# aanna0701/face-recognition-pytorch

Measured on AMD Instinct MI355X. Metric: train imgs/sec IR-50-layout ResNet50 + ArcFace/PartialFC head, 112x112, higher is better.
Workload: dtype bf16

## Files before the change

face-recognition-pytorch_amd/frhip/csrc/head.hip:

```cpp
#include "igemm_nt.h"
#include "margin_shared.h"
#include "frhip.h"

namespace frhip {

struct MarginConstEx : MarginConst { float m3, thr; };

constexpr int MG_ARC = 0, MG_ARC_EASY = 1, MG_COS = 2, MG_ROWS = 3;
struct MarginRows { float s, eps; const float* m_ang; const float* m_add; };
template <int MK, bool FILT> struct MarginArgOf { typedef MarginConstEx type; };
template <> struct MarginArgOf<MG_ARC, false> { typedef MarginConst type; };
template <> struct MarginArgOf<MG_ROWS, false> { typedef MarginRows type; };
template <int MK, bool FILT>
using MarginArg = typename MarginArgOf<MK, FILT>::type;

template <typename T>
__global__ __launch_bounds__(256) void l2norm_rows_kernel(const float* __restrict__ x, T* __restrict__ xhat,
                                                          float* __restrict__ norms, int rows, int D, float eps) {
    const int row = blockIdx.x * 4 + (threadIdx.x >> 6), lane = threadIdx.x & 63;
    if (row >= rows) return;
    const float* xr = x + (size_t)row * D;
    float ss = 0.f;
    for (int j = lane * 4; j < D; j += 256) {
        const f32x4_t v = *reinterpret_cast<const f32x4_t*>(xr + j);
// ... 124 lines not shown
                    if (cls == lab && mrow) {
                        ztarget[m] = zz;
                        if constexpr (SUB) tsub[m] = (int)((win[nt] >> (2 * (4 * mt + e))) & 3u);
                    }
                } else {
                    float d = 0.f;
                    if (cls < g.Nout && mrow) {
                        const float p = __expf(zz - gm) * gs;
                        bool inside;
                        if constexpr (MK == MG_ROWS) inside = raw >= tlo && raw <= thi;
                        else inside = raw >= -1.f && raw <= 1.f && !filtered;
                        d = inside ? (p - (cls == lab ? 1.f : 0.f)) * gscale * mc.s * slope : 0.f;
                    }
                    acc[nt][mt][e] = d;
                }
            }
        if (FWD) {
            vmax = lane_max_bit5(lane_max_bit4(vmax));
            float vs = 0.f;
            const float vref = vmax == -INFINITY ? 0.f : vmax;
#pragma unroll
            for (int nt = 0; nt < 4; ++nt)
#pragma unroll
                for (int e = 0; e < 4; ++e) vs += __expf(z[nt][e] - vref);
            vs = lane_sum_bit5(lane_sum_bit4(vs));
            if (fg == 0 && mrow) {
                part_max[(size_t)group * g.M + m] = vmax;
                part_sum[(size_t)group * g.M + m] = vs;
            }
        }
    }
}

template <typename T>
__device__ __forceinline__ void head_store_tile(const NtGeom& g, NtMainloop<T, 2, 2>& ml, char* smem, int m0, int n0, T* o, int ldt,
                                                int ncols, T* ot, int ldtt) {
    constexpr int P = NtTile<T, 2, 2>::template stage_pitch<T>();
    constexpr int EPV = 16 / (int)sizeof(T), LPR = 64 / EPV, RPI = 64 / LPR;
    const char* mine = ml.template stage_out<T>(smem);
    const int lane = lane_id(), chunk = lane % LPR, rsub = lane / LPR;
    const int n = n0 + chunk * EPV;
    for (int it = 0; it < 64 / RPI; ++it) {
        const int row = it * RPI + rsub, m = m0 + row;
        if (m < g.M && n < ncols)
            *reinterpret_cast<Vec16<T>*>(o + (size_t)m * ldt + n) = *reinterpret_cast<const Vec16<T>*>(mine + row * P + chunk * 16);
    }
    if (ot) {
        const int cls = n0 + lane;
        if (cls < g.Nout) {
#pragma unroll
            for (int v = 0; v < 64 / EPV; ++v) {
                Vec16<T> tv;
#pragma unroll
                for (int e = 0; e < EPV; ++e) tv.v[e] = *reinterpret_cast<const T*>(mine + (v * EPV + e) * P + lane * (int)sizeof(T));
                const int mcol = m0 + v * EPV;
                if (mcol < ldtt) *reinterpret_cast<Vec16<T>*>(ot + (size_t)cls * ldtt + mcol) = tv;
            }
        }
    }
}

template <typename T, bool FWD, int MK, bool FILT>
__global__ __launch_bounds__(256, 2) void head_kernel(NtGeom g, const void* __restrict__ ehat,
                                                             const void* __restrict__ what, const int* __restrict__ labels,
                                                             MarginArg<MK, FILT> mc, float* __restrict__ part_max,
                                                             float* __restrict__ part_sum, float* __restrict__ ztarget,
                                                             const float* __restrict__ rowmax, const float* __restrict__ rowsum,
                                                             float gscale, const float* __restrict__ upstream,
                                                             void* __restrict__ dt, int ldt, void* __restrict__ dtt, int ldtt,
                                                             int mtiles, int ntiles) {
    typedef NtTile<T, 2, 2> Tile;
    extern __shared__ __attribute__((aligned(16))) char smem[];
    const uint32_t lin = xcd_remap(blockIdx.x, gridDim.x);
    const int mtile = (int)(lin % (uint32_t)mtiles), ntile = (int)(lin / (uint32_t)mtiles);
    NtMainloop<T, 2, 2> ml;
    ml.run(g, ehat, what, smem, mtile, ntile, 0, g.ksteps);

    const int lane = lane_id(), wave = wave_id();
    const int wm = wave >> 1, wn = wave & 1;
    const int m0 = mtile * Tile::BM + wm * 64, n0 = ntile * Tile::BN + wn * 64;
    head_epilogue<FWD, MK, FILT, false>(lane, g, ml.acc, nullptr, m0, n0, ntile * 2 + wn, labels, mc, part_max, part_sum, ztarget, nullptr,
                                        rowmax, rowsum, gscale, upstream);
    if (!FWD) head_store_tile<T>(g, ml, smem, m0, n0, reinterpret_cast<T*>(dt), ldt, ldt, reinterpret_cast<T*>(dtt), ldtt);
}

constexpr int HEAD_SUB_MAX = 4;

template <typename T, bool FWD, int MK, bool FILT>
__global__ __launch_bounds__(256, 2) void head_sub_kernel(NtGeom g, const void* __restrict__ ehat,
                                                                 const void* __restrict__ what, const int* __restrict__ labels,
                                                                 MarginArg<MK, FILT> mc, int K, float* __restrict__ part_max,
                                                                 float* __restrict__ part_sum, float* __restrict__ ztarget,
                                                                 int* __restrict__ tsub, const float* __restrict__ rowmax,
                                                                 const float* __restrict__ rowsum, float gscale,
                                                                 const float* __restrict__ upstream, void* __restrict__ dt, int ldt,
                                                                 int ldp, void* __restrict__ dtt, int ldtt, int mtiles, int ntiles) {
    typedef NtTile<T, 2, 2> Tile;
    extern __shared__ __attribute__((aligned(16))) char smem[];
    const uint32_t lin = xcd_remap(blockIdx.x, gridDim.x);
    const int mtile = (int)(lin % (uint32_t)mtiles), ntile = (int)(lin / (uint32_t)mtiles);
    NtMainloop<T, 2, 2> ml;
    f32x4_t best[4][4];
    uint32_t win[4] = {0u, 0u, 0u, 0u};
    for (int k = 0; k < K; ++k) {
        if (k) __syncthreads();
        ml.run(g, ehat, reinterpret_cast<const char*>(what) + (size_t)k * g.b_bytes, smem, mtile, ntile, 0, g.ksteps);
#pragma unroll
        for (int nt = 0; nt < 4; ++nt)
#pragma unroll
            for (int mt = 0; mt < 4; ++mt)
#pragma unroll
                for (int e = 0; e < 4; ++e) {
                    const float v = ml.acc[nt][mt][e];
                    if (k == 0) best[nt][mt][e] = v;
                    else if (v > best[nt][mt][e]) {
                        best[nt][mt][e] = v;
                        win[nt] = (win[nt] & ~(3u << (2 * (4 * mt + e)))) | ((uint32_t)k << (2 * (4 * mt + e)));
                    }
                }
    }

    const int lane = lane_id(), wave = wave_id();
    const int wm = wave >> 1, wn = wave & 1;
    const int m0 = mtile * Tile::BM + wm * 64, n0 = ntile * Tile::BN + wn * 64;
    head_epilogue<FWD, MK, FILT, true>(lane, g, best, win, m0, n0, ntile * 2 + wn, labels, mc, part_max, part_sum, ztarget, tsub, rowmax,
                                       rowsum, gscale, upstream);
    if (!FWD)
        for (int k = 0; k < K; ++k) {
#pragma unroll
            for (int nt = 0; nt < 4; ++nt)
#pragma unroll
                for (int mt = 0; mt < 4; ++mt)
#pragma unroll
                    for (int e = 0; e < 4; ++e)
                        ml.acc[nt][mt][e] = ((win[nt] >> (2 * (4 * mt + e))) & 3u) == (uint32_t)k ? best[nt][mt][e] : 0.f;
            head_store_tile<T>(g, ml, smem, m0, n0, reinterpret_cast<T*>(dt) + (size_t)k * ldp, ldt, ldp,
                               dtt ? reinterpret_cast<T*>(dtt) + (size_t)k * g.Nout * ldtt : nullptr, ldtt);
        }
}

__global__ __launch_bounds__(256) void head_rowreduce_kernel(const float* __restrict__ part_max, const float* __restrict__ part_sum,
                                                             int ngroups, int N, float* __restrict__ rowmax, float* __restrict__ rowsum) {
    __shared__ float smax[16][17], ssum[16][17];
    const int ml = threadIdx.x & 15, gl = threadIdx.x >> 4;
    const int m = blockIdx.x * 16 + ml;
    float mx = -INFINITY, s = 0.f;
    if (m < N) {
        for (int gq = gl; gq < ngroups; gq += 16) {
            const float pm = part_max[(size_t)gq * N + m], ps = part_sum[(size_t)gq * N + m];
            if (pm > mx) { s = s * __expf(mx - pm) + ps; mx = pm; }
            else if (pm > -INFINITY) s += ps * __expf(pm - mx);
        }
    }
    smax[gl][ml] = mx; ssum[gl][ml] = s;
    __syncthreads();
    if (gl == 0 && m < N) {
        float M = -INFINITY;
#pragma unroll
        for (int k = 0; k < 16; ++k) M = fmaxf(M, smax[k][ml]);
        float S = 0.f;
#pragma unroll
        for (int k = 0; k < 16; ++k) if (smax[k][ml] > -INFINITY) S += ssum[k][ml] * __expf(smax[k][ml] - M);
        rowmax[m] = M; rowsum[m] = S;
    }
}

__global__ void head_rescale_kernel(float* __restrict__ rowsum, const float* __restrict__ local_max,
                                    const float* __restrict__ global_max, int N) {
    const int m = blockIdx.x * blockDim.x + threadIdx.x;
    if (m < N) rowsum[m] *= __expf(local_max[m] - global_max[m]);
}

__global__ void head_target_prob_kernel(const float* __restrict__ ztarget, const int* __restrict__ labels,
                                        const float* __restrict__ rowmax, const float* __restrict__ rowsum,
                                        float* __restrict__ q, int N) {
    const int m = blockIdx.x * blockDim.x + threadIdx.x;
    if (m < N) q[m] = labels[m] >= 0 ? __expf(ztarget[m] - rowmax[m]) / rowsum[m] : 0.f;
}

__global__ void head_pack_stats_kernel(const float* __restrict__ ztarget, const int* __restrict__ labels,
                                       const float* __restrict__ rowmax, const float* __restrict__ rowsum,
                                       float* __restrict__ packed, int N) {
    const int m = blockIdx.x * blockDim.x + threadIdx.x;
    if (m < N) {
// ... 20 lines not shown

__global__ void head_loss_kernel(const float* __restrict__ q, int N, float* __restrict__ loss) {
    __shared__ float red[256];
    float acc = 0.f;
    for (int m = threadIdx.x; m < N; m += 256) acc += logf(fmaxf(q[m], 1e-30f));
    red[threadIdx.x] = acc;
    __syncthreads();
    for (int d = 128; d > 0; d >>= 1) { if (threadIdx.x < d) red[threadIdx.x] += red[threadIdx.x + d]; __syncthreads(); }
    if (threadIdx.x == 0) loss[0] = -red[0] / (float)N;
}

struct HeadMargin { int mk; bool filt; MarginConstEx ex; MarginRows rows; };

template <int MK, bool FILT>
static MarginArg<MK, FILT> margin_arg(const HeadMargin& hm) {
    if constexpr (MK == MG_ROWS) return hm.rows;
    else return hm.ex;
}

struct HeadArgs {
    const void *ehat, *what;
    const int* labels;
    float *pmax, *psum, *zt;
    int* tsub;
    const float *rmax, *rsum;
    float gscale;
    const float* upstream;
    void* dt;
    int ldt, ldp;
    void* dtt;
    int ldtt;
};

template <typename T, bool FWD, int MK, bool FILT>
static int head_launch_mk(const NtGeom& g, const HeadArgs& a, const HeadMargin& hm, int K, hipStream_t stream) {
    typedef NtTile<T, 2, 2> Tile;
    const int mtiles = (g.M + Tile::BM - 1) / Tile::BM, ntiles = (g.Nout + Tile::BN - 1) / Tile::BN;
    const int lds = Tile::template lds_bytes<T>();
    const MarginArg<MK, FILT> mc = margin_arg<MK, FILT>(hm);
    auto plain = head_kernel<T, FWD, MK, FILT>;
    auto sub = head_sub_kernel<T, FWD, MK, FILT>;
    const char* who = K ? "head_sub" : "head";
    if (set_dynamic_lds(K ? reinterpret_cast<const void*>(sub) : reinterpret_cast<const void*>(plain), lds, who)) return FRHIP_ELAUNCH;
    if (K)
        hipLaunchKernelGGL(sub, dim3(mtiles * ntiles), dim3(256), lds, stream, g, a.ehat, a.what, a.labels, mc, K, a.pmax, a.psum, a.zt,
                           a.tsub, a.rmax, a.rsum, a.gscale, a.upstream, a.dt, a.ldt, a.ldp, a.dtt, a.ldtt, mtiles, ntiles);
    else
        hipLaunchKernelGGL(plain, dim3(mtiles * ntiles), dim3(256), lds, stream, g, a.ehat, a.what, a.labels, mc, a.pmax, a.psum, a.zt,
                           a.rmax, a.rsum, a.gscale, a.upstream, a.dt, a.ldt, a.dtt, a.ldtt, mtiles, ntiles);
    return check_launch(who);
}

template <bool FWD>
static int head_launch(int dtype, const NtGeom& g, const HeadArgs& a, const HeadMargin& hm, int K, hipStream_t stream) {
#define HEAD_VARIANT(MKV, FV) \
    if (hm.mk == MKV && hm.filt == FV) \
        return dtype == FRHIP_DT_BF16 ? head_launch_mk<bf16_t, FWD, MKV, FV>(g, a, hm, K, stream) \
                                      : head_launch_mk<float, FWD, MKV, FV>(g, a, hm, K, stream);
    HEAD_VARIANT(MG_ARC, false)
    HEAD_VARIANT(MG_ARC, true)
    HEAD_VARIANT(MG_ARC_EASY, false)
    HEAD_VARIANT(MG_ARC_EASY, true)
    HEAD_VARIANT(MG_COS, false)
    HEAD_VARIANT(MG_COS, true)
    HEAD_VARIANT(MG_ROWS, false)
#undef HEAD_VARIANT
    set_error("head: unknown margin variant %d", hm.mk);
    return FRHIP_EINVAL;
}

static int head_geom(NtGeom& g, int dtype, int n, int cl, int d, bool sub, int K, const char* who) {
    if (sub && (K < 1 || K > HEAD_SUB_MAX)) {
        set_error("%s: %d sub-centres per class (1 .. %d are supported)", who, K, HEAD_SUB_MAX);
        return FRHIP_EINVAL;
    }
    const int es = dtype == FRHIP_DT_BF16 ? 2 : 4, bke = NT_ROWB / es;
    if ((dtype != FRHIP_DT_BF16 && dtype != FRHIP_DT_F32) || n <= 0 || cl <= 0 || d <= 0 || (d % bke)) {
        set_error("%s: unsupported shape/dtype (n=%d classes=%d d=%d dtype=%d; d must be a multiple of %d)", who, n, cl, d, dtype, bke);
        return FRHIP_EINVAL;
    }
    if (1LL * cl * d * es > 0x7fffffffLL || 1LL * n * d * es > 0x7fffffffLL) { set_error("%s: operand exceeds 2 GiB", who); return FRHIP_EINVAL; }
    if (sub && 1LL * K * cl * d * es > 0x7fffffffLL) { set_error("%s: %d planes of %d classes exceed 2 GiB", who, K, cl); return FRHIP_EINVAL; }
    g.H = 1; g.W = 1; g.C = d; g.Ho = 1; g.Wo = 1; g.R = 1; g.S = 1; g.stride = 1; g.pad = 0; g.mode = 0;
    g.M = n; g.Nout = cl; g.Ktot = d; g.ksteps = d / bke; g.ksteps_per_split = g.ksteps;
    g.a_bytes = (uint32_t)(1LL * n * d * es); g.b_bytes = (uint32_t)(1LL * cl * d * es);
    g.par_a = -1; g.par_b = -1; g.hc = 0; g.wc = 0; g.par_r0 = 0; g.par_s0 = 0;
    return FRHIP_OK;
}

static int head_pitches(int dtype, int n, int cl, bool sub, int K, int ldt, int ldp, const void* dtt, int ldtt, const char* who) {
    const int epv = dtype == FRHIP_DT_BF16 ? 8 : 4;
    if (sub && (ldp < cl || (ldp % epv) || 1LL * ldt < 1LL * K * ldp || (ldt % epv))) {
        set_error("%s: bad dT pitches (row pitch %d, plane pitch %d, %d planes of %d classes)", who, ldt, ldp, K, cl);
        return FRHIP_EINVAL;
    }
    if (!sub && (ldt < cl || (ldt % epv))) { set_error("%s: bad dT pitch %d", who, ldt); return FRHIP_EINVAL; }
    if (dtt && (ldtt < n || (ldtt % epv))) { set_error("%s: bad transposed pitch %d", who, ldtt); return FRHIP_EINVAL; }
    return FRHIP_OK;
}

static int margin_desc(const frhip_margin_t* mg, HeadMargin& hm, const char* who) {
    if (!margin_desc_ok(mg)) {
        set_error("%s: bad margin descriptor (kind=%d thr=%g)", who, mg ? mg->kind : -1, mg ? (double)mg->filter_thr : 0.0);
        return FRHIP_EINVAL;
    }
    const bool arc = mg->kind == FRHIP_MARGIN_ARCFACE;
    static_cast<MarginConst&>(hm.ex) = margin_const(mg->s, arc ? mg->m : 0.f);
    hm.ex.m3 = arc ? 0.f : mg->m;
    hm.ex.thr = mg->filter_thr;
    hm.mk = arc ? (mg->easy ? MG_ARC_EASY : MG_ARC) : MG_COS;
    hm.filt = mg->filter_thr > 0.f;
    return FRHIP_OK;
}

static int margin_desc(const frhip_margin_rows_t* mg, HeadMargin& hm, const char* who) {
    if (!margin_rows_desc_ok(mg)) {
        set_error("%s: bad per-row margin descriptor (null pointer, or eps outside (0, 0.5))", who);
        return FRHIP_EINVAL;
    }
    hm.rows.s = mg->s; hm.rows.eps = mg->eps; hm.rows.m_ang = mg->m_ang; hm.rows.m_add = mg->m_add;
    hm.mk = MG_ROWS;
    hm.filt = false;
    return FRHIP_OK;
}

template <typename D>
static int head_fwd_impl(const char* who, int dtype, const void* ehat, const void* what, const int* labels, int n, int classes, int d,
                         bool sub, int K, const D* margin, float* part_max, float* part_sum, float* ztarget, int* tsub, float* rowmax,
                         float* rowsum, hipStream_t stream) {
    NtGeom g;
    HeadMargin hm = {};
    int rc = head_geom(g, dtype, n, classes, d, sub, K, who);
    if (rc || (rc = margin_desc(margin, hm, who))) return rc;
    HeadArgs a = {};
    a.ehat = ehat; a.what = what; a.labels = labels; a.pmax = part_max; a.psum = part_sum; a.zt = ztarget; a.tsub = tsub;
    if ((rc = head_launch<true>(dtype, g, a, hm, sub ? K : 0, stream))) return rc;
    hipLaunchKernelGGL(head_rowreduce_kernel, dim3((n + 15) / 16), dim3(256), 0, stream, part_max, part_sum,
                       frhip_head_groups(classes), n, rowmax, rowsum);
    char tag[64];
    snprintf(tag, sizeof(tag), "%s/rowreduce", who);
    return check_launch(tag);
}

template <typename D>
static int head_bwd_dt_impl(const char* who, int dtype, const void* ehat, const void* what, const int* labels, int n, int classes, int d,
                            bool sub, int K, const D* margin, const float* rowmax, const float* rowsum, float gscale,
                            const float* upstream, void* dt, int ldt, int ldp, void* dtt, int ldtt, hipStream_t stream) {
    NtGeom g;
    HeadMargin hm = {};
    int rc = head_geom(g, dtype, n, classes, d, sub, K, who);
    if (rc || (rc = head_pitches(dtype, n, classes, sub, K, ldt, ldp, dtt, ldtt, who)) || (rc = margin_desc(margin, hm, who))) return rc;
    HeadArgs a = {};
    a.ehat = ehat; a.what = what; a.labels = labels; a.rmax = rowmax; a.rsum = rowsum; a.gscale = gscale; a.upstream = upstream;
    a.dt = dt; a.ldt = ldt; a.ldp = ldp; a.dtt = dtt; a.ldtt = ldtt;
    return head_launch<false>(dtype, g, a, hm, sub ? K : 0, stream);
}

__device__ __forceinline__ double block_sum_f64(double v, double* red) {
#pragma unroll
    for (int d = 1; d < 64; d <<= 1) v += __shfl_xor(v, d);
    __syncthreads();
    if ((threadIdx.x & 63) == 0) red[threadIdx.x >> 6] = v;
    __syncthreads();
    double r = 0.0;
    for (int w = 0; w < (int)(blockDim.x >> 6); ++w) r += red[w];
    return r;
}

__device__ __forceinline__ double safe_norm(float x) { return (double)fminf(fmaxf(x, 0.001f), 100.f); }

__global__ __launch_bounds__(1024) void adaface_margins_kernel(const float* __restrict__ norms, int n, double m, double h, double t_alpha,
                                                               double eps, int update, float* __restrict__ batch_mean,
                                                               float* __restrict__ batch_std, float* __restrict__ m_ang,
                                                               float* __restrict__ m_add) {
// ... 3 lines not shown
    const double mean = block_sum_f64(acc, red) / (double)n;
    acc = 0.0;
    for (int i = threadIdx.x; i < n; i += blockDim.x) {
        const double dv = safe_norm(norms[i]) - mean;
        acc += dv * dv;
    }
    const double sd = sqrt(block_sum_f64(acc, red) / (double)(n - 1));
    double bm = (double)batch_mean[0], bs = (double)batch_std[0];
    if (update) { bm = t_alpha * mean + (1.0 - t_alpha) * bm; bs = t_alpha * sd + (1.0 - t_alpha) * bs; }
    __syncthreads();
    if (update && threadIdx.x == 0) { batch_mean[0] = (float)bm; batch_std[0] = (float)bs; }
    for (int i = threadIdx.x; i < n; i += blockDim.x) {
        const double k = fmin(fmax(h * (safe_norm(norms[i]) - bm) / (bs + eps), -1.0), 1.0);
        m_ang[i] = (float)(-m * k);
        m_add[i] = (float)(m + m * k);
    }
}

}

using namespace frhip;

extern "C" int frhip_adaface_margins(const float* norms, int n, double m, double h, double t_alpha, double eps, int update,
                                     float* batch_mean, float* batch_std, float* m_ang, float* m_add, hipStream_t stream) {
    if (n < 2 || !norms || !batch_mean || !batch_std || !m_ang || !m_add) {
        set_error("frhip_adaface_margins: needs n >= 2 norms (n=%d) and non-null norms, batch_mean, batch_std, m_ang, m_add", n);
        return FRHIP_EINVAL;
    }
    hipLaunchKernelGGL(adaface_margins_kernel, dim3(1), dim3(n > 256 ? 1024 : 256), 0, stream, norms, n, m, h, t_alpha, eps, update,
                       batch_mean, batch_std, m_ang, m_add);
    return check_launch("frhip_adaface_margins");
}

extern "C" int frhip_head_sub_max(void) { return HEAD_SUB_MAX; }

extern "C" int frhip_head_groups(int num_classes) { return ((num_classes + 127) / 128) * 2; }

extern "C" int frhip_head_fwd_ex(int dtype, const void* ehat, const void* what, const int* labels, int n, int classes,
                                 int d, const frhip_margin_t* margin, float* part_max, float* part_sum, float* ztarget,
                                 float* rowmax, float* rowsum, hipStream_t stream) {
    return head_fwd_impl("frhip_head_fwd", dtype, ehat, what, labels, n, classes, d, false, 1, margin, part_max, part_sum, ztarget, nullptr,
                         rowmax, rowsum, stream);
}

extern "C" int frhip_head_fwd(int dtype, const void* ehat, const void* what, const int* labels, int n, int classes,
                              int d, float s, float m, float* part_max, float* part_sum, float* ztarget,
                              float* rowmax, float* rowsum, hipStream_t stream) {
    const frhip_margin_t mg = {FRHIP_MARGIN_ARCFACE, 0, s, m, 0.f};
    return frhip_head_fwd_ex(dtype, ehat, what, labels, n, classes, d, &mg, part_max, part_sum, ztarget, rowmax, rowsum, stream);
}

extern "C" int frhip_head_fwd_rows(int dtype, const void* ehat, const void* what, const int* labels, int n, int classes,
                                   int d, const frhip_margin_rows_t* margin, float* part_max, float* part_sum, float* ztarget,
                                   float* rowmax, float* rowsum, hipStream_t stream) {
    return head_fwd_impl("frhip_head_fwd_rows", dtype, ehat, what, labels, n, classes, d, false, 1, margin, part_max, part_sum, ztarget,
                         nullptr, rowmax, rowsum, stream);
}

extern "C" int frhip_head_fwd_sub(int dtype, const void* ehat, const void* what, const int* labels, int n, int classes, int d,
                                  int subcenters, const frhip_margin_t* margin, float* part_max, float* part_sum, float* ztarget,
                                  int* tsub, float* rowmax, float* rowsum, hipStream_t stream) {
    return head_fwd_impl("frhip_head_fwd_sub", dtype, ehat, what, labels, n, classes, d, true, subcenters, margin, part_max, part_sum,
                         ztarget, tsub, rowmax, rowsum, stream);
}

extern "C" int frhip_head_fwd_sub_rows(int dtype, const void* ehat, const void* what, const int* labels, int n, int classes, int d,
// ... 90 lines not shown
```

include/frhip.h:

```cpp
#ifndef FRHIP_H
#define FRHIP_H
#include <stddef.h>
#include <stdint.h>

#ifdef __cplusplus
extern "C" {
#endif

#ifndef FRHIP_STREAM_T
#define FRHIP_STREAM_T
#ifdef __HIP_PLATFORM_AMD__
#include <hip/hip_runtime_api.h>
typedef hipStream_t frhip_stream_t;
#else
typedef void* frhip_stream_t;
#endif
#endif

#define FRHIP_OK 0
#define FRHIP_EINVAL (-1)
#define FRHIP_ELAUNCH (-2)
#define FRHIP_DT_BF16 0
#define FRHIP_DT_F32 1

const char* frhip_last_error(void);
int frhip_abi_version(void);
int frhip_spin(long long ticks, frhip_stream_t stream);

int frhip_nt_block_m(int k);
int frhip_conv_stat_rows(int dtype, int m, int k, int h, int w, int c, int r, int s, int stride, int pad);
int frhip_set_wgrad_taps9(int enabled);
int frhip_set_conv_halo(int enabled);
int frhip_set_halo_wide_dirs(int dirs);
int frhip_set_epi_lean(int enabled);
int frhip_set_ew_batch(int enabled);
int frhip_set_nt_tile(int tile);
int frhip_conv_fwd_affine(int dtype, const void* x, const void* w, void* y, const float* scale, const float* shift, int relu,
                          const void* residual, int n, int h, int wd, int c, int k, int r, int s, int stride, int pad,
                          frhip_stream_t stream);
int frhip_conv_fwd(int dtype, const void* x, const void* w, void* y, float* stats_partial,
                   int n, int h, int wd, int c, int k, int r, int s, int stride, int pad, frhip_stream_t stream);
int frhip_conv_dgrad(int dtype, const void* dy, const void* wt, void* dx, const void* residual,
                     int n, int h, int wd, int c, int k, int r, int s, int stride, int pad, frhip_stream_t stream);
int frhip_dgrad_stat_rows(int dtype, int n, int h, int wd, int c, int k, int r, int s, int stride, int pad);
int frhip_conv_dgrad_bnred(int dtype, const void* dy, const void* wt, void* dx, const void* residual,
                           const void* y_bn, const float* mean, const float* invstd, const float* mask_scale,
                           const float* mask_shift, float* stats_partial, int n, int h, int wd, int c, int k,
                           int r, int s, int stride, int pad, frhip_stream_t stream);
int frhip_conv_dgrad_fused(int dtype, const void* dy, const void* wt, void* dx, const void* residual, int residual_stride,
                           const void* y_bn, const float* mean, const float* invstd, const float* mask_scale,
                           const float* mask_shift, float* stats_partial, int n, int h, int wd, int c, int k,
                           int r, int s, int stride, int pad, frhip_stream_t stream);
int frhip_conv_dgrad_fused_rs(int dtype, const void* dy, const void* wt, void* dx, const void* residual, int residual_stride,
                              const void* y_bn, const float* mean, const float* invstd, const float* mask_scale,
                              const float* mask_shift, const float* rowscale, int rows_per, float keep_scale,
                              float* stats_partial, int n, int h, int wd, int c, int k, int r, int s, int stride, int pad,
                              frhip_stream_t stream);
int frhip_conv_wgrad(int dtype, const void* dy, const void* x, float* dw, int n, int h, int w, int c,
                     int k, int r, int s, int stride, int pad, int splits, float* workspace, size_t workspace_bytes,
                     frhip_stream_t stream);
int frhip_conv_wgrad_chain_ok(int dtype, int n, int h, int w, int c, int k, int r, int s, int stride, int pad);
int frhip_conv_wgrad_chain(int dtype, const void* dy, const void* x, int n, int h, int w, int c, int k, float* slabs,
                           size_t slab_bytes, float* prev_dw, const float* prev_slabs, int prev_k, int prev_c, int prev_splits,
                           int* splits_out, frhip_stream_t stream);
int frhip_conv_wgrad_chain_finish(float* dw, float* slabs, int k, int c, int splits, frhip_stream_t stream);
int frhip_linear_fwd(int dtype, const void* a, const void* w, const float* bias, void* out, void* act_out,
                     float* stats_partial, int m, int n, int k, frhip_stream_t stream);
int frhip_linear_dgrad_gelu(int dtype, const void* dy, const void* wt, const void* pre, void* dx, float* stats_partial,
// ... 45 lines not shown
int frhip_cast_from_f32(int dtype, const float* src, void* dst, size_t n, frhip_stream_t stream);
int frhip_cast_to_f32(int dtype, const void* src, float* dst, size_t n, frhip_stream_t stream);

int frhip_stem_im2col(int dtype, const float* x, void* col, int b, int h, int w, int stride, frhip_stream_t stream);
int frhip_bn_relu_maxpool_fwd(int dtype, const void* y, const float* scale, const float* shift, void* out,
                              uint8_t* argmax, int b, int h, int w, int c, frhip_stream_t stream);
int frhip_maxpool_bwd(int dtype, const void* dpool, const uint8_t* argmax, void* da, int b, int h, int w,
                      int c, frhip_stream_t stream);

int frhip_pack_wt(int dtype, const float* w, void* wt, int k, int rs, int c, frhip_stream_t stream);
int frhip_transpose2d(int dtype_in, int dtype_out, const void* in, void* out, int rows, int cols, int ld_out,
                      frhip_stream_t stream);
int frhip_pack_stem(int dtype, const float* w, void* wp, int k, int kin, int kp, frhip_stream_t stream);
int frhip_unpack_stem_grad(const float* dwp, float* dw, int k, int kin, int kp, frhip_stream_t stream);
int frhip_fc_permute(int dtype, const float* w, void* wp, int nout, int c, int hw, frhip_stream_t stream);
int frhip_fc_unpermute_grad(const float* dwp, float* dw, int nout, int c, int hw, frhip_stream_t stream);
int frhip_pfc_sample_max_local(void);
int frhip_pfc_sample(const int64_t* labels, int n, long long class_start, int num_local, const float* u, int num_sample,
                     int64_t* index_out, int* rel_out, int64_t* n_positive, frhip_stream_t stream);
int frhip_gather_rows(const float* src, const int64_t* index, float* dst, int n, int d, frhip_stream_t stream);
int frhip_scatter_rows(const float* src, const int64_t* index, float* dst, int n, int d, frhip_stream_t stream);

int frhip_head_dw_ok(int dtype, int n, int classes, int d);
int frhip_head_dw(int dtype, const void* dt, int ldt, const void* ehat, const void* what, const float* wnorm, float* dw,
                  int n, int classes, int d, float out_scale, frhip_stream_t stream);
int frhip_l2norm_rows(int dtype, const float* x, void* xhat, float* norms, int rows, int d, float eps,
                      frhip_stream_t stream);
int frhip_l2norm_bwd(int dtype, const float* dxhat, const void* xhat, const float* norms, float* dx,
                     int rows, int d, float out_scale, frhip_stream_t stream);
int frhip_head_groups(int num_classes);
int frhip_head_fwd(int dtype, const void* ehat, const void* what, const int* labels, int n, int classes,
                   int d, float s, float m, float* part_max, float* part_sum, float* ztarget,
                   float* rowmax, float* rowsum, frhip_stream_t stream);
int frhip_head_rescale(float* rowsum, const float* local_max, const float* global_max, int n, frhip_stream_t stream);
int frhip_head_target_prob(const float* ztarget, const int* labels, const float* rowmax, const float* rowsum,
                           float* q, int n, frhip_stream_t stream);
int frhip_head_pack_stats(const float* ztarget, const int* labels, const float* rowmax, const float* rowsum,
                          float* packed, int n, frhip_stream_t stream);
int frhip_head_merge_stats(const float* gathered, int world_size, int n, float* rowmax, float* rowsum, float* q,
                           frhip_stream_t stream);
int frhip_head_loss(const float* q, int n, float* loss, frhip_stream_t stream);
int frhip_head_bwd_dt(int dtype, const void* ehat, const void* what, const int* labels, int n, int classes,
                      int d, float s, float m, const float* rowmax, const float* rowsum, float gscale,
                      const float* upstream, void* dt, int ldt, void* dtt, int ldtt, frhip_stream_t stream);

#define FRHIP_MARGIN_ARCFACE 0
#define FRHIP_MARGIN_COSFACE 1
typedef struct { int kind; int easy; float s, m, filter_thr; } frhip_margin_t;
int frhip_head_fwd_ex(int dtype, const void* ehat, const void* what, const int* labels, int n, int classes,
                      int d, const frhip_margin_t* margin, float* part_max, float* part_sum, float* ztarget,
                      float* rowmax, float* rowsum, frhip_stream_t stream);
int frhip_head_bwd_dt_ex(int dtype, const void* ehat, const void* what, const int* labels, int n, int classes,
                         int d, const frhip_margin_t* margin, const float* rowmax, const float* rowsum, float gscale,
                         const float* upstream, void* dt, int ldt, void* dtt, int ldtt, frhip_stream_t stream);

typedef struct { float s, eps; const float* m_ang; const float* m_add; } frhip_margin_rows_t;
int frhip_adaface_margins(const float* norms, int n, double m, double h, double t_alpha, double eps, int update, float* batch_mean,
                          float* batch_std, float* m_ang, float* m_add, frhip_stream_t stream);
int frhip_head_fwd_rows(int dtype, const void* ehat, const void* what, const int* labels, int n, int classes,
                        int d, const frhip_margin_rows_t* margin, float* part_max, float* part_sum, float* ztarget,
                        float* rowmax, float* rowsum, frhip_stream_t stream);
int frhip_head_bwd_dt_rows(int dtype, const void* ehat, const void* what, const int* labels, int n, int classes,
                           int d, const frhip_margin_rows_t* margin, const float* rowmax, const float* rowsum, float gscale,
                           const float* upstream, void* dt, int ldt, void* dtt, int ldtt, frhip_stream_t stream);

int frhip_head_sub_max(void);
// ... 165 lines not shown
```

Baseline: 23220.

## Add pipelined multi-M-tile head kernel with hoisted row loads and batched rowreduce

Adds a head_pipe_kernel in which each block walks a run of consecutive M tiles for one class tile. It double-buffers LDS so the first k-step of the next M tile is staged while the current tile's epilogue and store run. Labels, rowmax and rowsum are loaded once per row ahead of the epilogue, and the upstream scale is folded in up front. The row-reduce kernel now batches its partial max/sum loads for more memory-level parallelism. This adds LDS pressure and enlarges the kernel, and the head is only a small part of full ResNet50 training.

After: 23330, median of 6. Within noise of the previous version (+0.5%).

```diff
diff --git a/face-recognition-pytorch_amd/frhip/csrc/head.hip b/face-recognition-pytorch_amd/frhip/csrc/head.hip
--- a/face-recognition-pytorch_amd/frhip/csrc/head.hip
+++ b/face-recognition-pytorch_amd/frhip/csrc/head.hip
@@ -180,6 +180,146 @@
     }
 }
 
+struct HeadRows { int lab[4]; float gm[4], gs[4]; };
+
+template <bool FUSED>
+__device__ __forceinline__ float arc_cos_tm(float t, float sin_t, float cos_m, float sin_m) {
+    if constexpr (FUSED) return fmaf(t, cos_m, -__fmul_rn(sin_t, sin_m));
+    else return __fsub_rn(__fmul_rn(t, cos_m), __fmul_rn(sin_t, sin_m));
+}
+
+template <bool FWD>
+__device__ __forceinline__ void head_rows_load(HeadRows& r, int lane, const NtGeom& g, int m0, const int* labels, const float* rowmax,
+                                               const float* rowsum) {
+#pragma unroll
+    for (int mt = 0; mt < 4; ++mt) {
+        const int m = m0 + mt * 16 + (lane & 15);
+        const bool mrow = m < g.M;
+        r.lab[mt] = mrow ? labels[m] : -1;
+        r.gm[mt] = 0.f; r.gs[mt] = 1.f;
+        if (!FWD && mrow) { r.gm[mt] = rowmax[m]; r.gs[mt] = 1.f / rowsum[m]; }
+    }
+}
+
+template <bool FWD, int MK, bool FILT, bool SUB>
+__device__ __forceinline__ void head_epilogue_hoisted(int lane, const NtGeom& g, f32x4_t (&acc)[4][4], const uint32_t* win, int m0, int n0,
+                                                      int group, const HeadRows& rows, MarginArg<MK, FILT> mc, float* part_max,
+                                                      float* part_sum, float* ztarget, int* tsub, float gscale) {
+    const int fi = lane & 15, fg = lane >> 4;
+#pragma unroll
+    for (int mt = 0; mt < 4; ++mt) {
+        const int m = m0 + mt * 16 + fi;
+        const bool mrow = m < g.M;
+        const int lab = rows.lab[mt];
+        const float gm = rows.gm[mt], gs = rows.gs[mt];
+        [[maybe_unused]] float tlo, thi;
+        if constexpr (MK == MG_ROWS) { tlo = -1.f + mc.eps; thi = 1.f - mc.eps; }
+        if constexpr (SUB)
+            if (FWD && group == 0 && fg == 0 && mrow && lab < 0) tsub[m] = -1;
+        const int rel = lab - n0;
+        const int slot = (lab >= 0 && (unsigned)rel < 64u && ((rel >> 2) & 3) == fg) ? (((rel >> 4) << 2) | (rel & 3)) : -1;
+        float tval = 0.f;
+        if (slot >= 0) {
+            float raw = 0.f;
+            [[maybe_unused]] uint32_t w = 0u;
+#pragma unroll
+            for (int nt = 0; nt < 4; ++nt)
+#pragma unroll
+                for (int e = 0; e < 4; ++e)
+                    if (slot == nt * 4 + e) {
+                        raw = acc[nt][mt][e];
+                        if constexpr (SUB) w = (win[nt] >> (2 * (4 * mt + e))) & 3u;
+                    }
+            float t;
+            if constexpr (MK == MG_ROWS) t = fminf(fmaxf(raw, tlo), thi);
+            else t = fminf(fmaxf(raw, -1.f), 1.f);
+            float slope = 1.f;
+            if constexpr (MK == MG_ARC) {
+                const float sin_t = sqrtf(fmaf(-t, t, 1.f));
+                if (t > mc.theta) { slope = mc.cos_m + t * mc.sin_m / sin_t; t = arc_cos_tm<FWD && !FILT>(t, sin_t, mc.cos_m, mc.sin_m); }
+                else t = t - mc.sinmm;
+            } else if constexpr (MK == MG_ARC_EASY) {
+                const float sin_t = sqrtf(fmaf(-t, t, 1.f));
+                if (t > 0.f) { slope = mc.cos_m + t * mc.sin_m / sin_t; t = arc_cos_tm<FWD && !FILT>(t, sin_t, mc.cos_m, mc.sin_m); }
+            } else if constexpr (MK == MG_ROWS) {
+                t = rows_margin_target(t, mc.m_ang[m], mc.m_add[m], mc.eps, slope);
+            } else {
+                t = t - mc.m3;
+            }
+            const float zz = t * mc.s;
+            if (FWD) {
+                tval = (lab < g.Nout) ? zz : -INFINITY;
+                ztarget[m] = zz;
+                if constexpr (SUB) tsub[m] = (int)w;
+            } else if (lab < g.Nout) {
+                const float p = __expf(zz - gm) * gs;
+                bool inside;
+                if constexpr (MK == MG_ROWS) inside = raw >= tlo && raw <= thi;
+                else inside = raw >= -1.f && raw <= 1.f;
+                tval = inside ? (p - 1.f) * gscale * mc.s * slope : 0.f;
+            }
+        }
+        float z[4][4];
+#pragma unroll
+        for (int nt = 0; nt < 4; ++nt)
+#pragma unroll
+            for (int e = 0; e < 4; ++e) {
+                const int cls = n0 + nt * 16 + 4 * fg + e;
+                const float raw = acc[nt][mt][e];
+                float t;
+                if constexpr (MK == MG_ROWS) t = fminf(fmaxf(raw, tlo), thi);
+                else t = fminf(fmaxf(raw, -1.f), 1.f);
+                bool filtered = false;
+                if constexpr (FILT) {
+                    if (t > mc.thr) { t = 0.f; filtered = true; }
+                }
+                const float zz = t * mc.s;
+                if (FWD) {
+                    z[nt][e] = (cls < g.Nout) ? zz : -INFINITY;
+                } else {
+                    float d = 0.f;
+                    if (cls < g.Nout && mrow) {
+                        const float p = __expf(zz - gm) * gs;
+                        bool inside;
+                        if constexpr (MK == MG_ROWS) inside = raw >= tlo && raw <= thi;
+                        else inside = raw >= -1.f && raw <= 1.f && !filtered;
+                        d = inside ? p * gscale * mc.s : 0.f;
+                    }
+                    acc[nt][mt][e] = d;
+                }
+            }
+        if (slot >= 0) {
+#pragma unroll
+            for (int nt = 0; nt < 4; ++nt)
+#pragma unroll
+                for (int e = 0; e < 4; ++e)
+                    if (slot == nt * 4 + e) {
+                        if (FWD) z[nt][e] = tval;
+                        else acc[nt][mt][e] = tval;
+                    }
+        }
+        if (FWD) {
+            float vmax = -INFINITY;
+#pragma unroll
+            for (int nt = 0; nt < 4; ++nt)
+#pragma unroll
+                for (int e = 0; e < 4; ++e) vmax = fmaxf(vmax, z[nt][e]);
+            vmax = lane_max_bit5(lane_max_bit4(vmax));
+            float vs = 0.f;
+            const float vref = vmax == -INFINITY ? 0.f : vmax;
+#pragma unroll
+            for (int nt = 0; nt < 4; ++nt)
+#pragma unroll
+                for (int e = 0; e < 4; ++e) vs += __expf(z[nt][e] - vref);
+            vs = lane_sum_bit5(lane_sum_bit4(vs));
+            if (fg == 0 && mrow) {
+                part_max[(size_t)group * g.M + m] = vmax;
+                part_sum[(size_t)group * g.M + m] = vs;
+            }
+        }
+    }
+}
+
 template <typename T>
 __device__ __forceinline__ void head_store_tile(const NtGeom& g, NtMainloop<T, 2, 2>& ml, char* smem, int m0, int n0, T* o, int ldt,
                                                 int ncols, T* ot, int ldtt) {
@@ -208,7 +348,7 @@
     }
 }
 
-template <typename T, bool FWD, int MK, bool FILT>
+template <typename T, bool FWD, int MK, bool FILT, bool HOIST>
 __global__ __launch_bounds__(256, 2) void head_kernel(NtGeom g, const void* __restrict__ ehat,
                                                              const void* __restrict__ what, const int* __restrict__ labels,
                                                              MarginArg<MK, FILT> mc, float* __restrict__ part_max,
@@ -227,14 +367,163 @@
     const int lane = lane_id(), wave = wave_id();
     const int wm = wave >> 1, wn = wave & 1;
     const int m0 = mtile * Tile::BM + wm * 64, n0 = ntile * Tile::BN + wn * 64;
-    head_epilogue<FWD, MK, FILT, false>(lane, g, ml.acc, nullptr, m0, n0, ntile * 2 + wn, labels, mc, part_max, part_sum, ztarget, nullptr,
-                                        rowmax, rowsum, gscale, upstream);
+    if constexpr (HOIST) {
+        HeadRows rows;
+        head_rows_load<FWD>(rows, lane, g, m0, labels, rowmax, rowsum);
+        if (!FWD && upstream) gscale *= upstream[0];
+        head_epilogue_hoisted<FWD, MK, FILT, false>(lane, g, ml.acc, nullptr, m0, n0, ntile * 2 + wn, rows, mc, part_max, part_sum, ztarget,
+                                                    nullptr, gscale);
+    } else
+        head_epilogue<FWD, MK, FILT, false>(lane, g, ml.acc, nullptr, m0, n0, ntile * 2 + wn, labels, mc, part_max, part_sum, ztarget, nullptr,
+                                            rowmax, rowsum, gscale, upstream);
     if (!FWD) head_store_tile<T>(g, ml, smem, m0, n0, reinterpret_cast<T*>(dt), ldt, ldt, reinterpret_cast<T*>(dtt), ldtt);
 }
 
+#ifndef FRHIP_HEAD_ABLATE
+#define FRHIP_HEAD_ABLATE 0
+#endif
+
+template <typename T, bool FWD>
+struct HeadPipe {
+    typedef NtTile<T, 2, 2> Tile;
+    static constexpr bool XSTORE = FWD || sizeof(T) == 2;
+    static constexpr int STORE_BYTES = Tile::WAVES * Tile::WROWS * Tile::template stage_pitch<T>();
+    static constexpr int S1_OFF = (!FWD && XSTORE) ? STORE_BYTES : Tile::STAGE_BYTES;
+    static constexpr int LDS_BYTES = FWD ? 2 * Tile::STAGE_BYTES
+                                         : (S1_OFF + Tile::STAGE_BYTES > STORE_BYTES ? S1_OFF + Tile::STAGE_BYTES : STORE_BYTES);
+    __device__ static __forceinline__ int store_off(int cur) { return (XSTORE && cur) ? Tile::STAGE_BYTES : 0; }
+    static_assert(S1_OFF >= Tile::STAGE_BYTES && (FWD || !XSTORE || STORE_BYTES <= S1_OFF) &&
+                  (FWD || (XSTORE ? Tile::STAGE_BYTES : 0) + STORE_BYTES <= LDS_BYTES), "the store tile fits beside the stage in flight");
+};
+
+template <typename T, bool FWD, int MK, bool FILT>
+__global__ __launch_bounds__(256, 2) void head_pipe_kernel(NtGeom g, const void* __restrict__ ehat, const void* __restrict__ what,
+                                                           const int* __restrict__ labels, MarginArg<MK, FILT> mc,
+                                                           float* __restrict__ part_max, float* __restrict__ part_sum,
+                                                           float* __restrict__ ztarget, const float* __restrict__ rowmax,
+                                                           const float* __restrict__ rowsum, float gscale,
+                                                           const float* __restrict__ upstream, void* __restrict__ dt, int ldt,
+                                                           void* __restrict__ dtt, int ldtt, int mtiles, int run) {
+    typedef NtTile<T, 2, 2> Tile;
+    typedef HeadPipe<T, FWD> Pipe;
+    typedef typename Mma<T>::Frag Frag;
+    constexpr int BM = Tile::BM, BN = Tile::BN;
+    extern __shared__ __attribute__((aligned(16))) char smem[];
+    const int mchunks = (mtiles + run - 1) / run;
+    const uint32_t lin = xcd_remap(blockIdx.x, gridDim.x);
+    const int mchunk = (int)(lin % (uint32_t)mchunks), ntile = (int)(lin / (uint32_t)mchunks);
+    const int mt_begin = mchunk * run, mt_end = min(mtiles, mt_begin + run);
+    const int lane = lane_id(), wave = wave_id();
+    const int wm = wave >> 1, wn = wave & 1;
+    const int fi = lane & 15, fg = lane >> 4;
+    if (!FWD && upstream) gscale *= upstream[0];
+
+    const __amdgpu_buffer_rsrc_t ra = make_rsrc(ehat, g.a_bytes);
+    const __amdgpu_buffer_rsrc_t rb = make_rsrc(what, g.b_bytes);
+    const int sub = lane >> 3;
+    const uint32_t chunk_bytes = (uint32_t)(((lane & 7) ^ sub) * 16);
+    const uint32_t rowbytes = (uint32_t)g.Ktot * (uint32_t)sizeof(T);
+    uint32_t brow_off[Tile::B_PIECES];
+#pragma unroll
+    for (int j = 0; j < Tile::B_PIECES; ++j) {
+        const int n = ntile * BN + (wave * Tile::B_PIECES + j) * 8 + sub;
+        brow_off[j] = (n < g.Nout) ? (uint32_t)n * rowbytes + chunk_bytes : OOB_OFFSET;
+    }
+    auto stage = [&](int buf, int mtile, int ks) {
+        if constexpr ((FRHIP_HEAD_ABLATE & 2) != 0) return;
+        char* sa = smem + (buf ? Pipe::S1_OFF : 0);
+        char* sb = sa + BM * NT_ROWB;
+        const uint32_t kb = (uint32_t)ks * (uint32_t)NT_ROWB;
+#pragma unroll
+        for (int j = 0; j < Tile::A_PIECES; ++j) {
+            const int m = mtile * BM + (wave * Tile::A_PIECES + j) * 8 + sub;
+            const uint32_t off = (m < g.M) ? (uint32_t)m * rowbytes + kb + chunk_bytes : OOB_OFFSET;
+            glds16(ra, sa + (wave * Tile::A_PIECES + j) * 1024, off);
+        }
+#pragma unroll
+        for (int j = 0; j < Tile::B_PIECES; ++j)
+            glds16(rb, sb + (wave * Tile::B_PIECES + j) * 1024, brow_off[j] == OOB_OFFSET ? OOB_OFFSET : brow_off[j] + kb);
+    };
+    NtMainloop<T, 2, 2> ml;
+    const int xoff = (wm * Tile::WROWS + fi) * NT_ROWB;
+    const int woff = BM * NT_ROWB + (wn * 64 + fi) * NT_ROWB;
+    const int sw = fi & 7;
+    auto compute = [&](int buf) {
+        if constexpr ((FRHIP_HEAD_ABLATE & 2) != 0) return;
+        const char* base = smem + (buf ? Pipe::S1_OFF : 0);
+#pragma unroll
+        for (int s = 0; s < RowFrag<T>::KSUB; ++s) {
+            Frag xf[4], wf[4];
+#pragma unroll
+            for (int t = 0; t < 4; ++t) wf[t] = RowFrag<T>::load(base + woff + t * 16 * NT_ROWB, fg, sw, s);
+#pragma unroll
+            for (int t = 0; t < 4; ++t) xf[t] = RowFrag<T>::load(base + xoff + t * 16 * NT_ROWB, fg, sw, s);
+#pragma unroll
+            for (int mt = 0; mt < 4; ++mt)
+#pragma unroll
+                for (int nt = 0; nt < 4; ++nt) Mma<T>::run(wf[nt], xf[mt], ml.acc[nt][mt]);
+        }
+    };
+    auto clear = [&]() {
+#pragma unroll
+        for (int i = 0; i < 4; ++i)
+#pragma unroll
+            for (int j = 0; j < 4; ++j) ml.acc[i][j] = f32x4_t{0.f, 0.f, 0.f, 0.f};
+    };
+
+    const int n0 = ntile * BN + wn * 64;
+    clear();
+    stage(0, mt_begin, 0);
+    asm volatile("s_waitcnt vmcnt(0)" ::: "memory");
+    __builtin_amdgcn_s_barrier();
+    int cur = 0;
+    for (int mtile = mt_begin; mtile < mt_end; ++mtile) {
+        for (int ks = 0; ks < g.ksteps - 1; ++ks) {
+            stage(cur ^ 1, mtile, ks + 1);
+            compute(cur);
+            asm volatile("s_waitcnt vmcnt(0)" ::: "memory");
+            __builtin_amdgcn_s_barrier();
+            cur ^= 1;
+        }
+        const bool more = mtile + 1 < mt_end;
+        const int m0 = mtile * BM + wm * 64;
+        HeadRows rows;
+        head_rows_load<FWD>(rows, lane, g, m0, labels, rowmax, rowsum);
+        if (Pipe::XSTORE && more) stage(cur ^ 1, mtile + 1, 0);
+        compute(cur);
+        if constexpr ((FRHIP_HEAD_ABLATE & 1) == 0)
+            head_epilogue_hoisted<FWD, MK, FILT, false>(lane, g, ml.acc, nullptr, m0, n0, ntile * 2 + wn, rows, mc, part_max, part_sum,
+                                                        ztarget, nullptr, gscale);
+        if constexpr (!FWD && (FRHIP_HEAD_ABLATE & 4) == 0)
+            head_store_tile<T>(g, ml, smem + Pipe::store_off(cur), m0, n0, reinterpret_cast<T*>(dt), ldt, ldt, reinterpret_cast<T*>(dtt), ldtt);
+        if constexpr ((FRHIP_HEAD_ABLATE & (FWD ? 1 : 4)) != 0) {
+            float keep = 0.f;
+#pragma unroll
+            for (int i = 0; i < 4; ++i)
+#pragma unroll
+                for (int j = 0; j < 4; ++j) keep += ml.acc[i][j][0] + ml.acc[i][j][1] + ml.acc[i][j][2] + ml.acc[i][j][3];
+            if (keep == 12345.678f && gscale == -7.f) (FWD ? part_max : reinterpret_cast<float*>(dt))[0] = keep;
+        }
+        if (more) {
+            clear();
+            if (Pipe::XSTORE) {
+                asm volatile("s_waitcnt vmcnt(0)" ::: "memory");
+                __builtin_amdgcn_s_barrier();
+                cur ^= 1;
+            } else {
+                __syncthreads();
+                stage(0, mtile + 1, 0);
+                asm volatile("s_waitcnt vmcnt(0)" ::: "memory");
+                __builtin_amdgcn_s_barrier();
+                cur = 0;
+            }
+        }
+    }
+}
+
 constexpr int HEAD_SUB_MAX = 4;
 
-template <typename T, bool FWD, int MK, bool FILT>
+template <typename T, bool FWD, int MK, bool FILT, bool HOIST>
 __global__ __launch_bounds__(256, 2) void head_sub_kernel(NtGeom g, const void* __restrict__ ehat,
                                                                  const void* __restrict__ what, const int* __restrict__ labels,
                                                                  MarginArg<MK, FILT> mc, int K, float* __restrict__ part_max,
@@ -271,8 +560,15 @@
     const int lane = lane_id(), wave = wave_id();
     const int wm = wave >> 1, wn = wave & 1;
     const int m0 = mtile * Tile::BM + wm * 64, n0 = ntile * Tile::BN + wn * 64;
-    head_epilogue<FWD, MK, FILT, true>(lane, g, best, win, m0, n0, ntile * 2 + wn, labels, mc, part_max, part_sum, ztarget, tsub, rowmax,
-                                       rowsum, gscale, upstream);
+    if constexpr (HOIST) {
+        HeadRows rows;
+        head_rows_load<FWD>(rows, lane, g, m0, labels, rowmax, rowsum);
+        if (!FWD && upstream) gscale *= upstream[0];
+        head_epilogue_hoisted<FWD, MK, FILT, true>(lane, g, best, win, m0, n0, ntile * 2 + wn, rows, mc, part_max, part_sum, ztarget, tsub,
+                                                   gscale);
+    } else
+        head_epilogue<FWD, MK, FILT, true>(lane, g, best, win, m0, n0, ntile * 2 + wn, labels, mc, part_max, part_sum, ztarget, tsub, rowmax,
+                                           rowsum, gscale, upstream);
     if (!FWD)
         for (int k = 0; k < K; ++k) {
 #pragma unroll
@@ -298,6 +594,46 @@
             const float pm = part_max[(size_t)gq * N + m], ps = part_sum[(size_t)gq * N + m];
             if (pm > mx) { s = s * __expf(mx - pm) + ps; mx = pm; }
             else if (pm > -INFINITY) s += ps * __expf(pm - mx);
+        }
+    }
+    smax[gl][ml] = mx; ssum[gl][ml] = s;
+    __syncthreads();
+    if (gl == 0 && m < N) {
+        float M = -INFINITY;
+#pragma unroll
+        for (int k = 0; k < 16; ++k) M = fmaxf(M, smax[k][ml]);
+        float S = 0.f;
+#pragma unroll
+        for (int k = 0; k < 16; ++k) if (smax[k][ml] > -INFINITY) S += ssum[k][ml] * __expf(smax[k][ml] - M);
+        rowmax[m] = M; rowsum[m] = S;
+    }
+}
+
+constexpr int ROWRED_ROWS = 8, ROWRED_BATCH = 16;
+
+__global__ __launch_bounds__(16 * ROWRED_ROWS) void head_rowreduce_batched_kernel(const float* __restrict__ part_max,
+                                                                                  const float* __restrict__ part_sum, int ngroups, int N,
+                                                                                  float* __restrict__ rowmax, float* __restrict__ rowsum) {
+    __shared__ float smax[16][ROWRED_ROWS + 1], ssum[16][ROWRED_ROWS + 1];
+    const int ml = threadIdx.x % ROWRED_ROWS, gl = threadIdx.x / ROWRED_ROWS;
+    const int m = blockIdx.x * ROWRED_ROWS + ml;
+    float mx = -INFINITY, s = 0.f;
+    if (m < N) {
+        for (int g0 = gl; g0 < ngroups; g0 += 16 * ROWRED_BATCH) {
+            float bm[ROWRED_BATCH], bs[ROWRED_BATCH];
+#pragma unroll
+            for (int j = 0; j < ROWRED_BATCH; ++j) {
+                const int gq = g0 + 16 * j;
+                const bool ok = gq < ngroups;
+                bm[j] = ok ? part_max[(size_t)gq * N + m] : -INFINITY;
+                bs[j] = ok ? part_sum[(size_t)gq * N + m] : 0.f;
+            }
+#pragma unroll
+            for (int j = 0; j < ROWRED_BATCH; ++j) {
+                const float pm = bm[j], ps = bs[j];
+                if (pm > mx) { s = s * __expf(mx - pm) + ps; mx = pm; }
+                else if (pm > -INFINITY) s += ps * __expf(pm - mx);
+            }
         }
     }
     smax[gl][ml] = mx; ssum[gl][ml] = s;
@@ -384,14 +720,28 @@
     int ldtt;
 };
 
-template <typename T, bool FWD, int MK, bool FILT>
+static int g_head_fast = 1;
+static int g_head_run = 2;
+
+template <typename T, bool FWD, int MK, bool FILT, bool HOIST>
 static int head_launch_mk(const NtGeom& g, const HeadArgs& a, const HeadMargin& hm, int K, hipStream_t stream) {
     typedef NtTile<T, 2, 2> Tile;
     const int mtiles = (g.M + Tile::BM - 1) / Tile::BM, ntiles = (g.Nout + Tile::BN - 1) / Tile::BN;
     const int lds = Tile::template lds_bytes<T>();
     const MarginArg<MK, FILT> mc = margin_arg<MK, FILT>(hm);
-    auto plain = head_kernel<T, FWD, MK, FILT>;
-    auto sub = head_sub_kernel<T, FWD, MK, FILT>;
+    if constexpr (HOIST) {
+        if (!K && g_head_run > 0) {
+            typedef HeadPipe<T, FWD> Pipe;
+            const int run = g_head_run < mtiles ? g_head_run : mtiles, mchunks = (mtiles + run - 1) / run;
+            auto pipe = head_pipe_kernel<T, FWD, MK, FILT>;
+            if (set_dynamic_lds(reinterpret_cast<const void*>(pipe), Pipe::LDS_BYTES, "head_pipe")) return FRHIP_ELAUNCH;
+            hipLaunchKernelGGL(pipe, dim3(mchunks * ntiles), dim3(256), Pipe::LDS_BYTES, stream, g, a.ehat, a.what, a.labels, mc, a.pmax,
+                               a.psum, a.zt, a.rmax, a.rsum, a.gscale, a.upstream, a.dt, a.ldt, a.dtt, a.ldtt, mtiles, run);
+            return check_launch("head_pipe");
+        }
+    }
+    auto plain = head_kernel<T, FWD, MK, FILT, HOIST>;
+    auto sub = head_sub_kernel<T, FWD, MK, FILT, HOIST>;
     const char* who = K ? "head_sub" : "head";
     if (set_dynamic_lds(K ? reinterpret_cast<const void*>(sub) : reinterpret_cast<const void*>(plain), lds, who)) return FRHIP_ELAUNCH;
     if (K)
@@ -406,9 +756,13 @@
 template <bool FWD>
 static int head_launch(int dtype, const NtGeom& g, const HeadArgs& a, const HeadMargin& hm, int K, hipStream_t stream) {
 #define HEAD_VARIANT(MKV, FV) \
-    if (hm.mk == MKV && hm.filt == FV) \
-        return dtype == FRHIP_DT_BF16 ? head_launch_mk<bf16_t, FWD, MKV, FV>(g, a, hm, K, stream) \
-                                      : head_launch_mk<float, FWD, MKV, FV>(g, a, hm, K, stream);
+    if (hm.mk == MKV && hm.filt == FV) { \
+        if (g_head_fast) \
+            return dtype == FRHIP_DT_BF16 ? head_launch_mk<bf16_t, FWD, MKV, FV, true>(g, a, hm, K, stream) \
+                                          : head_launch_mk<float, FWD, MKV, FV, true>(g, a, hm, K, stream); \
+        return dtype == FRHIP_DT_BF16 ? head_launch_mk<bf16_t, FWD, MKV, FV, false>(g, a, hm, K, stream) \
+                                      : head_launch_mk<float, FWD, MKV, FV, false>(g, a, hm, K, stream); \
+    }
     HEAD_VARIANT(MG_ARC, false)
     HEAD_VARIANT(MG_ARC, true)
     HEAD_VARIANT(MG_ARC_EASY, false)
@@ -474,6 +828,16 @@
     hm.mk = MG_ROWS;
     hm.filt = false;
     return FRHIP_OK;
+}
+
+static int head_rowreduce_launch(const char* who, const float* part_max, const float* part_sum, int ngroups, int n, float* rowmax,
+                                 float* rowsum, hipStream_t stream) {
+    if (g_head_fast)
+        hipLaunchKernelGGL(head_rowreduce_batched_kernel, dim3((n + ROWRED_ROWS - 1) / ROWRED_ROWS), dim3(16 * ROWRED_ROWS), 0, stream,
+                           part_max, part_sum, ngroups, n, rowmax, rowsum);
+    else
+        hipLaunchKernelGGL(head_rowreduce_kernel, dim3((n + 15) / 16), dim3(256), 0, stream, part_max, part_sum, ngroups, n, rowmax, rowsum);
+    return check_launch(who);
 }
 
 template <typename D>
@@ -487,11 +851,9 @@
     HeadArgs a = {};
     a.ehat = ehat; a.what = what; a.labels = labels; a.pmax = part_max; a.psum = part_sum; a.zt = ztarget; a.tsub = tsub;
     if ((rc = head_launch<true>(dtype, g, a, hm, sub ? K : 0, stream))) return rc;
-    hipLaunchKernelGGL(head_rowreduce_kernel, dim3((n + 15) / 16), dim3(256), 0, stream, part_max, part_sum,
-                       frhip_head_groups(classes), n, rowmax, rowsum);
     char tag[64];
     snprintf(tag, sizeof(tag), "%s/rowreduce", who);
-    return check_launch(tag);
+    return head_rowreduce_launch(tag, part_max, part_sum, frhip_head_groups(classes), n, rowmax, rowsum, stream);
 }
 
 template <typename D>
@@ -561,6 +923,27 @@
     return check_launch("frhip_adaface_margins");
 }
 
+extern "C" int frhip_set_head_fast(int enabled) {
+    const int old = g_head_fast;
+    if (enabled >= 0) g_head_fast = enabled ? 1 : 0;
+    return old;
+}
+
+extern "C" int frhip_set_head_run(int tiles) {
+    const int old = g_head_run;
+    if (tiles >= 0) g_head_run = tiles;
+    return old;
+}
+
+extern "C" int frhip_head_rowreduce(const float* part_max, const float* part_sum, int ngroups, int n, float* rowmax, float* rowsum,
+                                    hipStream_t stream) {
+    if (ngroups <= 0 || n <= 0 || !part_max || !part_sum || !rowmax || !rowsum) {
+        set_error("frhip_head_rowreduce: bad arguments (ngroups=%d n=%d, or a null pointer)", ngroups, n);
+        return FRHIP_EINVAL;
+    }
+    return head_rowreduce_launch("frhip_head_rowreduce", part_max, part_sum, ngroups, n, rowmax, rowsum, stream);
+}
+
 extern "C" int frhip_head_sub_max(void) { return HEAD_SUB_MAX; }
 
 extern "C" int frhip_head_groups(int num_classes) { return ((num_classes + 127) / 128) * 2; }
diff --git a/include/frhip.h b/include/frhip.h
--- a/include/frhip.h
+++ b/include/frhip.h
@@ -34,6 +34,8 @@
 int frhip_set_halo_wide_dirs(int dirs);
 int frhip_set_epi_lean(int enabled);
 int frhip_set_ew_batch(int enabled);
+int frhip_set_head_fast(int enabled);
+int frhip_set_head_run(int tiles);
 int frhip_set_nt_tile(int tile);
 int frhip_conv_fwd_affine(int dtype, const void* x, const void* w, void* y, const float* scale, const float* shift, int relu,
                           const void* residual, int n, int h, int wd, int c, int k, int r, int s, int stride, int pad,
@@ -145,6 +147,8 @@
 int frhip_head_fwd(int dtype, const void* ehat, const void* what, const int* labels, int n, int classes,
                    int d, float s, float m, float* part_max, float* part_sum, float* ztarget,
                    float* rowmax, float* rowsum, frhip_stream_t stream);
+int frhip_head_rowreduce(const float* part_max, const float* part_sum, int ngroups, int n, float* rowmax, float* rowsum,
+                         frhip_stream_t stream);
 int frhip_head_rescale(float* rowsum, const float* local_max, const float* global_max, int n, frhip_stream_t stream);
 int frhip_head_target_prob(const float* ztarget, const int* labels, const float* rowmax, const float* rowsum,
                            float* q, int n, frhip_stream_t stream);
```
